# embedded-software-laboratory/p-dmpc

Measured on AMD Instinct MI355X. Metric: MPC steps/sec (whole node) + p50 per-step plan latency, N vehicles H=8, higher is better.
Workload: dtype f64

## Files before the change

p-dmpc_amd/csrc/api.cpp:

```cpp
#include <hip/hip_runtime.h>

#include <algorithm>
#include <cmath>
#include <cstdio>
#include <cstdlib>
#include <chrono>
#include <cstring>
#include <limits>
#include <mutex>
#include <string>
#include <type_traits>
#include <vector>

#include "choice_host.hpp"
#include "handle.hpp"
#include "mpa_reach.hpp"
#include "reference_tree.hpp"
#include "sampled_launch.hpp"

namespace {

thread_local std::string g_err;

std::mutex g_lds_mutex;
uint32_t g_lds_high_water[64][4][2];

void set_launch_args(pdmpc_handle* h, const PackedStep& B, const LaunchPlan& plan, int first, int count, KernelArgs& a) {
    set_batch_args(h, B, plan.areas_in_lds, a);
    set_plan_args(h->tune, plan, a);
    a.dt = h->cfg.dt_seconds;
    a.max_nodes = h->arena.max_nodes;
    a.checker = h->cfg.checker;
    a.pred = B.dev.pred;
    a.done_flag = h->d_flag.p;
    a.epoch = h->epoch;
    a.first = first;
    a.arena = h->arena.view();
    a.soup_cap = B.soup_cap;
    a.cand_cap = B.cand_cap;
    a.tie_count = h->d_tie_count.p;
    if (h->tune.debug_progress && !h->progress) {
        if (hipHostMalloc((void**)&h->progress, (size_t)h->max_vehicles * 64 * 4, hipHostMallocMapped) != hipSuccess) h->progress = nullptr;
        if (h->progress) std::memset(h->progress, 0, (size_t)h->max_vehicles * 64 * 4);
    }
    a.progress = h->progress;
    a.bk_post = h->d_bk_post.p;
    a.help_board = h->d_help_board.p;
    a.help_verdict = h->d_help_verdict.p;
    a.help_finished = h->d_help_finished.p;
    h->launch_serial += 1;
    if (h->launch_serial == 0) h->launch_serial = 1;
    a.launch_id = h->launch_serial;
    a.n_searches = count;
}

int prepare_boards(pdmpc_handle* h, int count, uint32_t& fin_base) {
    fin_base = 0;
    if (!h->boards_dirty) {
        fin_base = h->help_fin_total;
        h->help_fin_total += (uint32_t)count;
    } else {
        HIPCHK(hipMemsetAsync(h->d_help_board.p, 0, (size_t)h->max_vehicles * PDMPC_HB_WORDS * sizeof(unsigned long long), h->stream));
        HIPCHK(hipMemsetAsync(h->d_help_finished.p, 0, 16 * sizeof(uint32_t), h->stream));
        h->help_fin_total = (uint32_t)count;
        h->boards_dirty = false;
    }
    return PDMPC_OK;
}

struct SearchLaunch {
    KernelArgs a{};

    int prepare(pdmpc_handle* h, const PackedStep& B, int first, int count, bool safe, LaunchPlan& plan) {
        const LaunchDims dims = launch_dims(h, B);
        int n_chained = 0;
        if (!safe && policy_reads_chained(h->tune, count, dims.n_cu, dims.device_share))
            for (int i = 0; i < count; ++i) n_chained += B.host.veh[first + i].n_pred > 0 ? 1 : 0;
        std::string err;
        int rc = plan_launch(h->tune, dims, kPlanSearch, count, n_chained, safe, plan, err);
        if (rc) return fail(rc, err);
        set_launch_args(h, B, plan, first, count, a);
        if (plan.n_helpers > 0 && (rc = prepare_boards(h, count, a.help_fin_base))) return rc;
        if (h->tune.debug_lds) fputs(format_bulk_layout(plan, count).c_str(), stderr);
        return PDMPC_OK;
    }

    int go(const pdmpc_handle* h, const LaunchPlan& plan) const {
        typedef int (*launcher_t)(const KernelArgs*, int, void*, uint32_t*);
        static const launcher_t launchers[4][2] = {{pdmpc_launch_bulk, pdmpc_launch_bulk_any},
                                                   {pdmpc_launch_bulk_wide, pdmpc_launch_bulk_wide_any},
                                                   {pdmpc_launch_bulk_sat, pdmpc_launch_bulk_sat_any},
                                                   {pdmpc_launch_bulk_compact, pdmpc_launch_bulk_compact_any}};
        const int variant = plan.variant, generic = plan.generic ? 1 : 0;
        int lrc = 0;
        for (int done = 0; done < a.n_searches && lrc == 0; done += plan.slice) {
            KernelArgs part = a;
            part.first = a.first + done;
            part.n_searches = std::min(plan.slice, a.n_searches - done);
            std::lock_guard<std::mutex> lock(g_lds_mutex);
            lrc = launchers[variant][generic](&part, part.n_searches, (void*)h->stream, &g_lds_high_water[h->cfg.device & 63][variant][generic]);
        }
        return lrc;
    }
};

template <class Launch>
int timed_launch(pdmpc_handle* h, const PackedStep& B, int first, int count, bool safe, LaunchKind kind) {
    LaunchPlan plan;
    Launch launch;
    int rc = launch.prepare(h, B, first, count, safe, plan);
    if (rc) return rc;
    if ((rc = h->timer.begin(h->stream, kind))) return rc;
    const int lrc = launch.go(h, plan);
    if (lrc != 0) {
        h->boards_dirty = true;
        char buf[256];
        snprintf(buf, sizeof buf, "kernel launch failed: %s (LDS %u B)", hipGetErrorString((hipError_t)lrc), plan.lds.total);
        return fail(PDMPC_ERR_HIP, buf);
    }
    if ((rc = h->timer.end(h->stream))) return rc;
    h->stats.lds_bytes = plan.lds.total;
    h->stats.lds_nodes = plan.NL;
    return PDMPC_OK;
}

int launch_range(pdmpc_handle* h, int first, int count, bool safe) {
    if (!h) return fail(PDMPC_ERR_INVALID, "null handle");
    PackedStep& B = h->banks[h->bank];
// ... 1133 lines not shown
```

p-dmpc_amd/csrc/bulk_search.hpp:

```cpp
#include <hip/hip_runtime.h>

#include "search_common.hpp"

#include "frontier_common.hpp"

#include "bk_shared.hpp"
#include "bk_helper.hpp"

#define BK_P2 3
#define BK_PER PDMPC_BK_PER
#define BK_FAST_PER 4

namespace {

__device__ __forceinline__ unsigned long long wg_scan_excl(unsigned long long v, lds_vu64* wsum, int lane, int wave, int n_waves, unsigned long long& total) {
    unsigned long long inc = v;
#pragma unroll
    for (int o = 1; o < PDMPC_WAVE; o <<= 1) {
        const unsigned long long t = __shfl_up(inc, o);
        inc += lane >= o ? t : 0ull;
    }
    if (lane == PDMPC_WAVE - 1) wsum[wave] = inc;
    __syncthreads();
    unsigned long long off = 0, tot = 0;
// ... 1492 lines not shown
                    if (bsel != 0u || scale == 0.0 || (to_mid ? cum <= 4u * fill : nn_near + cum <= OC - 64u)) break;
                    hi = lo + (hi - lo) / (double)FR_NBINS;
                }
                const bool all = bsel >= FR_NBINS - 1 || scale == 0.0;
                const double l_new = all ? inf : lo + (double)(bsel + 1u) / scale;
                if (tid == 0) {
                    if (from_mid) {
                        sh_st_d(sh, BK_MID_MIN, inf);
                    } else {
                        sh_st_d(sh, FR_FAR_MIN, inf);
                        sh_st_d(sh, FR_FAR_MAX, 0.0);
                    }
                    if (to_mid) {
                        sh_st_d(sh, BK_L_MID, all ? hi_src : l_new);
                    } else {
                        if (!from_mid) sh_st_d(sh, BK_L_MID, -1.0);
                        if (nn_near == 0u) {
                            sh_st_d(sh, FR_NEAR_MIN, inf);
                            sh_st_d(sh, FR_NEAR_MAX, 0.0);
                        }
                        const double l_far_new = (all && far_left != 0u) ? l_mid_old : l_new;
                        const double l_old = sh_ld_d(sh, FR_L_FAR);
                        sh_st_d(sh, FR_L_FAR, (nn_near != 0u && l_old > l_far_new && l_old < inf) ? l_old : l_far_new);
                    }
                }
                __syncthreads();
                load_l_mid();
                const double lo_c = lo, scale_c = scale;
                const uint32_t kept = fr_partition(
                    src_key, src_id, fn, wsum, n_waves, [&](double k, uint32_t i) -> int { return i == 0u ? -1 : (fr_bin(k, lo_c, scale_c) <= bsel ? 1 : 0); },
                    [&](int c, double k, uint32_t i) {
                        const unsigned long long b = __ballot(c == 1);
                        bool back = false;
                        if (b && to_mid) {
                            const uint32_t base = sh_add_uniform(sh, BK_MID_N, (uint32_t)__builtin_popcountll(b), lane);
                            if (c == 1) {
                                const uint32_t pos = base + lane_rank(b, lane);
                                mid_key[pos] = k;
                                mid_id[pos] = i;
                                mid_mn = k < mid_mn ? k : mid_mn;
                            }
                        } else if (b) {
                            const uint32_t base = sh_add_uniform(sh, FR_NEAR_N, (uint32_t)__builtin_popcountll(b), lane);
                            const uint32_t pos = base + lane_rank(b, lane);
                            const bool fits = c == 1 && pos < OC;
                            if (fits) {
                                near_key[pos] = k;
                                near_id[pos] = i;
                                near_mn = k < near_mn ? k : near_mn;
                                near_mx = k > near_mx ? k : near_mx;
                            }
                            back = c == 1 && !fits;
                        }
                        if (!to_mid) to_far(back, k, i);
                        if (c < 0 && i != 0u) {
                            if (from_mid) {
                                mid_mn = k < mid_mn ? k : mid_mn;
                            } else {
                                far_mn = k < far_mn ? k : far_mn;
                                far_mx = k > far_mx ? k : far_mx;
                            }
                        }
                    });
                flush_far();
                flush_near();
                const uint32_t extra = sh[SRC_N] - fn;
                for (uint32_t e = (uint32_t)tid; e < extra; e += (uint32_t)bd) {
                    src_key[kept + e] = src_key[fn + e];
                    src_id[kept + e] = src_id[fn + e];
                }
                asm volatile("s_waitcnt vmcnt(0)" ::: "memory");
                __syncthreads();
                if (tid == 0) {
                    sh[SRC_N] = kept + extra;
                    if (sh[FR_NEAR_N] > OC) sh[FR_NEAR_N] = OC;
                }
                __syncthreads();
            }
            nn_near = sh[FR_NEAR_N];
            BK_TICK(tk_refill)
        }

        BK_OPAQUE_TID
        if (nn_near <= (uint32_t)(BK_FAST_PER * PDMPC_WAVE)) {
            BK_TICK3(4)
            __syncthreads();
            if (wave == 0) {
                const double lo = sh_ld_d(sh, FR_NEAR_MIN), hi = sh_ld_d(sh, FR_NEAR_MAX);
                double kk[BK_FAST_PER];
                uint32_t ii[BK_FAST_PER];
#pragma unroll
                for (int j = 0; j < BK_FAST_PER; ++j) {
                    const uint32_t e = (uint32_t)j * PDMPC_WAVE + (uint32_t)lane;
                    kk[j] = e < nn_near ? near_key[e] : 0.0;
                    ii[j] = e < nn_near ? near_id[e] : 0u;
                }
                double thr = hi;
                if (nn_near > round_target) {
                    double a = lo, b = hi;
                    for (int it = 0; it < 48; ++it) {
                        const double mid = a + (b - a) * 0.5;
                        if (!(mid > a) || !(mid < b)) break;
                        uint32_t c = 0;
#pragma unroll
                        for (int j = 0; j < BK_FAST_PER; ++j) c += (uint32_t)__builtin_popcountll(__ballot(ii[j] != 0u && kk[j] <= mid));
                        if (c >= round_target) {
                            thr = mid;
                            b = mid;
                            if (c <= 2u * round_target + 16u) break;
                        } else {
                            a = mid;
                        }
                    }
                }
                const bool have_goal = best != 0u;
                const bool check_alive = sh[FR_EVER_INVAL] != 0u;
                const uint32_t epoch_now = sh[BK_ARRIVALS] & 0xffffu;
                ulonglong2* const wcache = (ulonglong2*)A.arena.walk + voff;
                uint32_t pk = 0, pr = 0, n_dead = 0, n_drop = 0;
#pragma unroll
                for (int j = 0; j < BK_FAST_PER; ++j) {
                    const double k = kk[j];
                    const uint32_t i = ii[j];
                    const bool sel = i != 0u && k <= thr;
                    const bool above = have_goal && k > bb;
                    const bool walk = sel && !above && (have_goal || check_alive);
                    if (sel && have_goal && k == bb) atomicOr((uint32_t*)&sh[FR_FLAGS], FRF_TIE);
                    int r = 1;
                    if (have_goal || check_alive) r = bk_classify_wave(F.glink, wcache, VS, F.gkey, gp_path, gp_mp, have_goal, check_alive, best, epoch_now, walk ? i : 0u, k, sh);
                    const int c = i == 0u ? -1 : (sel ? (above ? 3 : r) : 0);
                    const unsigned long long bk = __ballot(c == 0), br = __ballot(c == 1);
                    n_dead += (uint32_t)__builtin_popcountll(__ballot(c == 4));
                    n_drop += (uint32_t)__builtin_popcountll(__ballot(c == 3));
                    if (c == 0) {
                        const uint32_t pos = pk + lane_rank(bk, lane);
                        near_key[pos] = k;
                        near_id[pos] = i;
                        near_mn = k < near_mn ? k : near_mn;
                        near_mx = k > near_mx ? k : near_mx;
                    } else if (c == 1) {
                        const uint32_t pos = pr + lane_rank(br, lane);
                        ready[pos] = i;
                        r_flag[pos] = 0u;
                    }
                    pk += (uint32_t)__builtin_popcountll(bk);
                    pr += (uint32_t)__builtin_popcountll(br);
                }
                if (lane == 0) {
                    sh[FR_NEAR_N] = pk;
                    sh_st_d(sh, FR_NEAR_MIN, inf);
                    sh_st_d(sh, FR_NEAR_MAX, 0.0);
                    sh[FR_SEL_BIN] = pr;
                    if (n_dead) sh[FR_DEAD] = sh[FR_DEAD] + n_dead;
                    if (n_drop) sh[FR_DROPPED] = sh[FR_DROPPED] + n_drop;
                }
            }
            __syncthreads();
            Rn = sh[FR_SEL_BIN];
            BK_TICK3(5)
            BK_TICK(tk_select)
            continue;
        }
        {
            BK_TICK3(4)
            if (!(nn_near > round_target)) __syncthreads();
            const double lo = sh_ld_d(sh, FR_NEAR_MIN);
            double hi = sh_ld_d(sh, FR_NEAR_MAX);
            double kk[BK_PER];
            uint32_t ii[BK_PER];
#pragma unroll
            for (int j = 0; j < BK_PER; ++j) {
                const uint32_t e = (uint32_t)j * (uint32_t)bd + (uint32_t)tid;
                kk[j] = e < nn_near ? near_key[e] : 0.0;
                ii[j] = e < nn_near ? near_id[e] : 0u;
            }
            uint32_t bsel = BK_NB - 1;
            double scale = 0.0;
            const bool use_hist = nn_near > round_target;
            if (use_hist) {
                for (int zoom = 0; zoom < 8; ++zoom) {
                    scale = hi > lo ? (double)BK_NB / (hi - lo) : 0.0;
#pragma unroll
                    for (int j = 0; j < BK_PER; ++j)
                        if (ii[j]) __hip_atomic_fetch_add(&bins[bk_bin(kk[j], lo, scale)], 1u, __ATOMIC_RELAXED, __HIP_MEMORY_SCOPE_WORKGROUP);
                    __syncthreads();
                    uint32_t cum;
                    bk_select(bins, round_target, lane, bsel, cum);
                    if (cum <= 2u * round_target + 16u || scale == 0.0) break;
                    hi = lo + (hi - lo) / (double)BK_NB;
                    __syncthreads();
                    if (tid < BK_NB) bins[tid] = 0u;
                    __syncthreads();
                }
            }
            const bool have_goal = best != 0u;
            const bool check_alive = sh[FR_EVER_INVAL] != 0u;
            const uint32_t epoch_now = sh[BK_ARRIVALS] & 0xffffu;
            ulonglong2* const wcache = (ulonglong2*)A.arena.walk + voff;
            int cls[BK_PER];
            unsigned long long mine = 0;
            uint32_t n_dead = 0, n_drop = 0;
#pragma unroll
            for (int j = 0; j < BK_PER; ++j) {
                const double k = kk[j];
                const uint32_t i = ii[j];
                const uint32_t b = bk_bin(k, lo, scale);
                const bool sel = i != 0u && b <= bsel;
                const bool above = have_goal && k > bb;
                const bool walk = sel && !above && (have_goal || check_alive);
                if (sel && have_goal && k == bb) atomicOr((uint32_t*)&sh[FR_FLAGS], FRF_TIE);
                int r = 1;
                if (have_goal || check_alive) r = bk_classify_wave(F.glink, wcache, VS, F.gkey, gp_path, gp_mp, have_goal, check_alive, best, epoch_now, walk ? i : 0u, k, sh);
                cls[j] = i == 0u ? -1 : (sel ? (above ? 3 : r) : 0);
                mine += (cls[j] == 0 ? 1ull : 0ull) | (cls[j] == 1 ? (1ull << 32) : 0ull);
                n_dead += cls[j] == 4 ? 1u : 0u;
                n_drop += cls[j] == 3 ? 1u : 0u;
            }
            unsigned long long tot = 0;
            const unsigned long long base = wg_scan_excl(mine, wsum64 + 16, lane, wave, n_waves, tot);
            if (use_hist && tid < BK_NB) bins[tid] = 0u;
            const uint32_t n_keep = (uint32_t)(tot & 0xffffffffull), n_rdy = (uint32_t)(tot >> 32);
            if (tid == 0) {
                sh[FR_NEAR_N] = n_keep;
                sh_st_d(sh, FR_NEAR_MIN, inf);
                sh_st_d(sh, FR_NEAR_MAX, 0.0);
            }
            {
                uint32_t pk = (uint32_t)(base & 0xffffffffull), pr = (uint32_t)(base >> 32);
                bool over[BK_PER];
#pragma unroll
                for (int j = 0; j < BK_PER; ++j) {
                    over[j] = false;
                    if (cls[j] == 0) {
                        near_key[pk] = kk[j];
                        near_id[pk] = ii[j];
                        near_mn = kk[j] < near_mn ? kk[j] : near_mn;
                        near_mx = kk[j] > near_mx ? kk[j] : near_mx;
                        pk += 1u;
                    } else if (cls[j] == 1) {
                        if (pr < RC) {
                            ready[pr] = ii[j];
                            r_flag[pr] = 0u;
                        } else {
                            over[j] = true;
                        }
                        pr += 1u;
                    }
                }
                if (n_rdy > RC) {
#pragma unroll
                    for (int j = 0; j < BK_PER; ++j) to_far(over[j], kk[j], ii[j]);
                }
            }
            if (n_dead) sh_add(sh, FR_DEAD, n_dead);
            if (n_drop) sh_add(sh, FR_DROPPED, n_drop);
            Rn = n_rdy < RC ? n_rdy : RC;
            __syncthreads();
            BK_TICK3(5)
            BK_TICK(tk_select)
        }
    }

    int tid_r = tid_k, lane_r = lane_k;
    asm volatile("" : "+v"(tid_r), "+v"(lane_r));
    uint32_t nnodes_raw = sh[FR_NNODES];
    nnodes_raw = nnodes_raw < S.max_nodes ? nnodes_raw : S.max_nodes;
    __syncthreads();
    const bool pb_ran = pb_valid;
    if (!pb_valid) {
        R.n_popped = 0;
        R.n_expanded = nnodes_raw;
    }
    {
        const uint32_t nv = vs_copied ? 0u : (VS.NV < nnodes_raw ? VS.NV : nnodes_raw);
        for (uint32_t i = (uint32_t)tid_r; i < nv; i += (uint32_t)bd) VS.g[i] = VS.l[i];
    }
    {
        unsigned long long a = t_checks, b = t_pairs;
#pragma unroll
        for (int o = PDMPC_WAVE / 2; o > 0; o >>= 1) {
            a += __shfl_xor(a, o);
            b += __shfl_xor(b, o);
        }
        if (lane_r == 0) {
            atomicAdd(A.work_count + 0, a);
            atomicAdd(A.work_count + 1, b);
        }
    }
    if (tid_r == 0) {
        atomicAdd(P.counters + 2, (int)sh[BK_ARRIVALS]);
        atomicAdd(A.work_count + 2, (unsigned long long)sh[FR_PROCESSED]);
        atomicAdd(A.work_count + 3, (unsigned long long)sh[FR_ROUNDS]);
        A.tree_size[slot] = (int32_t)(nnodes_raw | PDMPC_TREE_FRONTIER | (tie_replayed ? PDMPC_TREE_REPLAYED : 0u));
    }
    if (tid_r == 0 && SW::debug_tail(A)) {
        double* dbg = X.O->path_nodes[PDMPC_HP_MAX];
        dbg[0] = (double)sh[FR_ROUNDS];
        dbg[1] = (double)sh[FR_PROCESSED];
        dbg[2] = (double)nnodes_raw;
        dbg[3] = (double)sh[FR_NEAR_N];
        dbg[4] = (double)(sh[FR_FAR_N] + sh[BK_MID_N]);
        dbg[5] = (double)sh[FR_FLAGS];
        dbg[6] = (double)sh[BK_ARRIVALS];
        dbg[7] = (double)(__builtin_amdgcn_s_memrealtime() - tk[TK_START]);
        for (int i = 0; i < 6; ++i) X.O->path_nodes[PDMPC_HP_MAX - 3][i] = (double)tk2[i];
        if (A.n_helpers > 0) {
            const unsigned long long sw = __hip_atomic_load(board + PDMPC_HB_SEATS, __ATOMIC_RELAXED, __HIP_MEMORY_SCOPE_AGENT);
            X.O->path_nodes[PDMPC_HP_MAX - 3][7] = (double)pdmpc_hb_seats_count(sw);
        }
        X.O->path_nodes[PDMPC_HP_MAX - 2][0] = (double)(tk[TK_START] - X.rt_kernel_start);
        X.O->path_nodes[PDMPC_HP_MAX - 2][1] = (double)tk[tk_p1];
        X.O->path_nodes[PDMPC_HP_MAX - 2][2] = (double)tk[tk_p2];
        X.O->path_nodes[PDMPC_HP_MAX - 2][3] = (double)tk[tk_p3];
        X.O->path_nodes[PDMPC_HP_MAX - 2][4] = (double)tk[tk_pb];
        X.O->path_nodes[PDMPC_HP_MAX - 2][5] = (double)tk[tk_refill];
        X.O->path_nodes[PDMPC_HP_MAX - 1][0] = (double)(tk[tk_work] + tk[tk_p1] + tk[tk_p2] + tk[tk_p3]);
        X.O->path_nodes[PDMPC_HP_MAX - 1][1] = (double)tk[tk_arrival];
        X.O->path_nodes[PDMPC_HP_MAX - 1][2] = (double)tk[tk_select];
        X.O->path_nodes[PDMPC_HP_MAX - 1][3] = (double)tk[tk_wait];
        X.O->path_nodes[PDMPC_HP_MAX - 1][4] = (double)(tk[TK_MARK] - tk[TK_START]);
        X.O->path_nodes[PDMPC_HP_MAX - 1][5] = (double)tk[tk_pub];
        X.O->path_nodes[PDMPC_HP_MAX - 1][6] = (double)__builtin_amdgcn_s_memrealtime();
        X.O->path_nodes[PDMPC_HP_MAX - 1][7] = (double)X.rt_kernel_start;
    }
    X.status = status;
    X.n_popped = (int)R.n_popped;
    X.path_ready = pb_ran && goal != 0u;
    X.goal = goal;
    X.nnodes = R.n_expanded;
    X.dep_timeout = dep_timeout;
    X.rec_valid = rec_valid && !dep_timeout;
    X.rec_written = rec_written;
    X.published = sh[BK_PUBLISHED] != 0u;
}

template <int NW, int CHECKER, class SW>
__device__ __forceinline__ void bulk_body(const KernelArgs& A) {
    if ((int)blockIdx.x < A.bk_helpers_first || (int)blockIdx.x >= A.bk_helpers_first + A.n_searches) {
        bulk_helper_body<CHECKER, SW>(A);
        return;
    }
    extern __shared__ __attribute__((aligned(16))) unsigned char smem[];
    Ctx X;
    const unsigned long long rt0 = __builtin_amdgcn_s_memrealtime();
    search_prologue<SW>(A, X, (LDS_AS unsigned char*)smem);
    X.rt_kernel_start = rt0;
    const int wave = X.wave;
    lds_u32* ref_ids = bk_misc(X.lsm)->ref_ids;
    bulk_search<NW, CHECKER, SW>(A, X, ref_ids);
    __syncthreads();
    if (wave != 0) return;
    {
        int l__ = X.lane;
        asm volatile("" : "+v"(l__));
        X.lane = l__;
    }
    if (!X.rec_valid) bk_write_record(A, X, X.goal, X.status, X.dep_timeout, (uint32_t)X.n_popped, X.nnodes, X.path_ready, ref_ids, X.rec_written, X.published, X.lane);
    bk_publish(A, X, X.status, X.dep_timeout);
    if (X.lane == 0 && A.n_helpers > 0) {
        __hip_atomic_store(A.help_board + (size_t)X.slot * PDMPC_HB_WORDS + PDMPC_HB_WANT, 0ull, __ATOMIC_RELAXED, __HIP_MEMORY_SCOPE_AGENT);
        atomicAdd(A.help_finished, 1u);
    }
}

}

#ifndef PDMPC_BULK_KERNEL_ATTR
#define PDMPC_BULK_KERNEL_ATTR
#endif
#define PDMPC_BULK_INSTANCE(NAME, LAUNCHER, NW, CHECKER, MAXWAVES, SW)                                                                   \
    extern "C" __global__ __launch_bounds__(PDMPC_WAVE * (MAXWAVES)) PDMPC_BULK_KERNEL_ATTR void NAME(const KernelArgs A) { bulk_body<NW, CHECKER, SW>(A); } \
    extern "C" int LAUNCHER(const KernelArgs* args, int count, void* stream, uint32_t* lds_high_water) {                                \
        if (count <= 0) return 0;                                                                                                        \
        typedef void (*kernel_t)(const KernelArgs);                                                                                      \
        kernel_t fn = NAME;                                                                                                              \
         \
        uint32_t& have = lds_high_water[0];                                                                                              \
        if (args->lds.total > have) {                                                                                                    \
            hipError_t e = hipFuncSetAttribute((const void*)fn, hipFuncAttributeMaxDynamicSharedMemorySize, (int)args->lds.total);       \
            if (e != hipSuccess) return (int)e;                                                                                          \
            have = args->lds.total;                                                                                                      \
        }                                                                                                                                \
        hipLaunchKernelGGL(fn, dim3(count + (args->n_helpers > 0 ? args->n_helpers : 0)), dim3(PDMPC_WAVE * args->n_waves), args->lds.total, (hipStream_t)stream, *args); \
        return (int)hipGetLastError();                                                                                                   \
    }
#define PDMPC_BULK_KERNEL(NAME, LAUNCHER, NW, CHECKER, MAXWAVES, KERNEL)                    \
    PDMPC_BULK_INSTANCE(NAME, LAUNCHER, NW, CHECKER, MAXWAVES, SwitchesProduct<KERNEL>)  \
    PDMPC_BULK_INSTANCE(NAME##_any, LAUNCHER##_any, NW, CHECKER, MAXWAVES, SwitchesFromArgs)
```

p-dmpc_amd/csrc/handle.hpp:

```cpp
#pragma once
#include <vector>

#include "hdv_host.hpp"
#include "hip_host.hpp"
#include "launch_plan.hpp"
#include "pdmpc_device.h"


struct Arenas {
    uint32_t max_nodes = 0;
    DevBuf<NodeRec> nodes;
    DevBuf<double> key, far_key, mid_key, pb_key, walk;
    DevBuf<unsigned long long> link;
    DevBuf<uint32_t> far_id, mid_id, pb_d, child0, vlist;
    DevBuf<uint8_t> vstate;
    template <class Self, class F>
    static void each(Self& a, int Hp, F&& f) {
        f(a.nodes, 1);
        f(a.key, 1);
        f(a.link, 1);
        f(a.vstate, 1);
        f(a.far_key, 1);
        f(a.far_id, 1);
        f(a.mid_key, 1);
        f(a.mid_id, 1);
        f(a.pb_key, 1);
        f(a.pb_d, 1);
        f(a.walk, 2);
        f(a.child0, 1);
        f(a.vlist, Hp + 1);
    }
    size_t bytes_per_node(int Hp) const {
        size_t sum = 0;
        each(*this, Hp, [&](const auto& b, int per) { sum += (size_t)per * sizeof *b.p; });
        return sum;
    }
    int alloc(int max_vehicles, uint32_t n, int Hp) {
        n = (n + 1u) & ~1u;
        const size_t tot = (size_t)max_vehicles * n;
        each(*this, Hp, [](auto& b, int) { b.release(); });
        max_nodes = 0;
        int bad = 0;
        each(*this, Hp, [&](auto& b, int per) { bad |= b.ensure_exact(tot * (size_t)per); });
        if (bad) return bad;
        max_nodes = n;
        return 0;
    }
    NodeArena view() const {
        return {nodes.p, key.p, link.p, vstate.p, far_key.p, far_id.p, mid_key.p, mid_id.p, pb_key.p, pb_d.p, walk.p, child0.p, vlist.p};
    }
};

enum LaunchKind : int32_t { kLaunchSearch = 2, kLaunchSampled = 3, kLaunchJoint = 4 };

struct BlobRegions {
    DevVehicle* veh = nullptr;
    int32_t* pred = nullptr;
    double* pts = nullptr;
};

struct PackedStep {
    PinnedBuf<unsigned char> h_blob;
    DevBuf<unsigned char> d_blob;
    BlobRegions host, dev;
    uint64_t staged_serial = ~0ull;
    int n_packed = 0;
    bool pack_failed = false;
    SampledBank sampled;
    int soup_cap = 0;
    int ll_cap = 0;
    int cand_cap = 0;
    std::vector<int64_t> lit_cols;
    std::vector<int32_t> perm;
    std::vector<int32_t> inv;
};

struct SoupKey {
    const void* p[13];
    int32_t c[6];
};

struct SoupTable {
    std::vector<SoupKey> keys;
    std::vector<int32_t> slot;
    std::vector<int32_t> table;
    static uint64_t hash(const SoupKey& k) {
        static_assert(sizeof(SoupKey) % 8 == 0, "SoupKey is hashed by 64-bit words");
        uint64_t hsh = 1469598103934665603ull;
        const uint64_t* w = (const uint64_t*)&k;
        for (size_t q = 0; q < sizeof(SoupKey) / 8; ++q) hsh = (hsh ^ w[q]) * 1099511628211ull;
        return hsh ^ (hsh >> 29);
    }
    void reset(int n) {
        size_t size = 64;
        while (size < (size_t)n * 2) size *= 2;
        keys.clear();
        slot.clear();
        table.assign(size, 0);
    }
    int find(const SoupKey& k, size_t& at) const {
        for (at = (size_t)hash(k) & (table.size() - 1); table[at] != 0; at = (at + 1) & (table.size() - 1)) {
            const int q = table[at] - 1;
            if (std::memcmp(&keys[(size_t)q], &k, sizeof k) == 0) return slot[(size_t)q];
        }
        return -1;
    }
    void insert(const SoupKey& k, int packed_in, size_t at) {
        keys.push_back(k);
        slot.push_back(packed_in);
        table[at] = (int32_t)keys.size();
    }
};

struct LaunchTimer {
    static constexpr size_t kMaxPairs = 4096;
    std::vector<std::pair<hipEvent_t, hipEvent_t>> events;
    size_t used = 0;
    double folded_ms = 0.0;
    int64_t folded_launches = 0;
    LaunchKind kind = kLaunchSampled;
    LaunchTimer() = default;
    LaunchTimer(const LaunchTimer&) = delete;
    LaunchTimer& operator=(const LaunchTimer&) = delete;
    ~LaunchTimer() { release(); }
    void release() {
        for (auto& ev : events) {
            (void)hipEventDestroy(ev.first);
            (void)hipEventDestroy(ev.second);
        }
        events.clear();
        used = 0;
    }
// ... 244 lines not shown
```

p-dmpc_amd/csrc/pdmpc_device.h:

```cpp
#ifndef PDMPC_DEVICE_H
#define PDMPC_DEVICE_H

#include <stdint.h>

#include "../../include/pdmpc.h"
#include "../../include/pdmpc_hdv.h"

#define PDMPC_WAVE 64
#define PDMPC_MAX_WAVES 16
#define PDMPC_MAX_WAVES_SAT 12
#define PDMPC_SH_WORDS 128

struct DevManPose {
    double dx, dy, dyaw;
    int32_t n_cols;
    int32_t pad;
};

struct DevVehicle {
    double x0, y0, yaw0;
    double ref_x[PDMPC_HP_MAX];
    double ref_y[PDMPC_HP_MAX];
    double v_ref[PDMPC_HP_MAX];
    int32_t trim0;
    int32_t n_pred;
    int32_t pred_off;
    int32_t ll_off, ll_len;
    int32_t lit_off[PDMPC_HP_MAX + 1];
    int32_t hdv_off[PDMPC_HP_MAX + 1];
    int32_t fb_off[PDMPC_HP_MAX + 1];
    uint32_t seed;
};

struct NodeRec {
    double x, y, yaw, g;
    double cs, sn;
    double h;
    uint32_t parent;
    uint32_t packed;
};
#define NODE_TRIM(p) ((int)((p) & 1023u))
#define NODE_K(p) ((int)(((p) >> 10) & 31u))
#define NODE_MAN(p) ((int)(((p) >> 15) & 4095u))
#define NODE_COLS(p) ((int)(((p) >> 27) & 15u))

struct LdsLayout {
    uint32_t mask, man_index, pose, area;
    uint32_t ref;
    uint32_t shape;
    uint32_t path;
    uint32_t soup;
    uint32_t cand;
    uint32_t vstate;
    uint32_t expand;
    uint32_t tree16;
    uint32_t rand;
    uint32_t nodes;
    uint32_t total;
    uint32_t bk_near_key, bk_near_id;
    uint32_t bk_ready;
    uint32_t bk_hist;
    uint32_t bk_misc;
    uint32_t bk_pshape;
    uint32_t reach_shared;
    uint32_t bk_reach;
    uint32_t reach;
};

struct LdsPathRegion {
    uint32_t path[PDMPC_HP_MAX + 2];
    int32_t soff[PDMPC_HP_MAX + 1];
    int32_t hoff[PDMPC_HP_MAX + 1];
    uint32_t shared[PDMPC_SH_WORDS];
    int32_t lit[PDMPC_HP_MAX];
};
#define PDMPC_LK_PATH_BYTES PDMPC_LK_ALIGN16((uint32_t)sizeof(LdsPathRegion))

#define PDMPC_LK_ALIGN16(x) (((x) + 15u) & ~15u)
#ifndef PDMPC_LK_WAVES
#define PDMPC_LK_WAVES PDMPC_MAX_WAVES
#endif
#ifndef PDMPC_LK_READY_CAP
#define PDMPC_LK_READY_CAP 2048u
#endif
#define PDMPC_LK_COMPACT_WAVES 8
#define PDMPC_LK_COMPACT_READY_CAP 512u
#define PDMPC_LK_COMPACT_BK_PER 2
#define PDMPC_LKX_THREADS(W) ((uint32_t)(W) * PDMPC_WAVE)
#define PDMPC_LKX_REF 0u
#define PDMPC_LKX_SHAPE (PDMPC_LKX_REF + 3u * PDMPC_HP_MAX * 8u)
#define PDMPC_LKX_PATH(W) (PDMPC_LKX_SHAPE + (uint32_t)(W) * (2u * PDMPC_VMAX + 1u) * 16u)
#define PDMPC_LKX_CAND(W) (PDMPC_LKX_PATH(W) + PDMPC_LK_PATH_BYTES)
#define PDMPC_LKX_EXPAND(W) (PDMPC_LKX_CAND(W) + PDMPC_LK_ALIGN16(12u * PDMPC_LKX_THREADS(W)))
#define PDMPC_LKX_NEAR_KEY(W) (PDMPC_LKX_EXPAND(W) + (2u * PDMPC_HP_MAX * PDMPC_HP_MAX) * 8u + 16u * 16u)
#define PDMPC_LKX_NEAR_ID(W, P) (PDMPC_LKX_NEAR_KEY(W) + PDMPC_LK_ALIGN16((uint32_t)(P) * PDMPC_LKX_THREADS(W) * 8u))
#define PDMPC_LKX_READY(W, P) (PDMPC_LKX_NEAR_ID(W, P) + PDMPC_LK_ALIGN16((uint32_t)(P) * PDMPC_LKX_THREADS(W) * 4u))
#define PDMPC_LKX_HIST(W, RC, P) (PDMPC_LKX_READY(W, P) + (uint32_t)(RC) * 8u)
#define PDMPC_LKX_MISC(W, RC, P) (PDMPC_LKX_HIST(W, RC, P) + 3072u * 4u)
#define PDMPC_LKX_PSHAPE(W, RC, P) (PDMPC_LKX_MISC(W, RC, P) + 2048u)
#define PDMPC_LKX_REACH(W, RC, P) (PDMPC_LKX_PSHAPE(W, RC, P) + PDMPC_LK_ALIGN16(PDMPC_HP_MAX * PDMPC_VMAX * 16u + PDMPC_HP_MAX * 4u + PDMPC_HP_MAX * 8u + PDMPC_HP_MAX * 4u))
#define PDMPC_LK_REACH_CNT (PDMPC_HP_MAX * 4u * 8u)
#define PDMPC_LK_REACH_STALE (PDMPC_LK_REACH_CNT + 3u * PDMPC_HP_MAX * 4u)
#define PDMPC_LK_REACH_SC (PDMPC_LK_REACH_STALE + 16u)
#define PDMPC_LK_REACH_ROOT (PDMPC_LK_REACH_SC + 32u)
#define PDMPC_LKX_FIXED_END(W, RC, P) (PDMPC_LKX_REACH(W, RC, P) + PDMPC_LK_REACH_ROOT + 64u)
#ifndef PDMPC_BK_PER
#define PDMPC_BK_PER 4
#endif
#define PDMPC_LK_REF PDMPC_LKX_REF
#define PDMPC_LK_SHAPE PDMPC_LKX_SHAPE
#define PDMPC_LK_PATH PDMPC_LKX_PATH(PDMPC_LK_WAVES)
#define PDMPC_LK_CAND PDMPC_LKX_CAND(PDMPC_LK_WAVES)
#define PDMPC_LK_EXPAND PDMPC_LKX_EXPAND(PDMPC_LK_WAVES)
#define PDMPC_LK_NEAR_KEY PDMPC_LKX_NEAR_KEY(PDMPC_LK_WAVES)
#define PDMPC_LK_NEAR_ID PDMPC_LKX_NEAR_ID(PDMPC_LK_WAVES, PDMPC_BK_PER)
#define PDMPC_LK_READY PDMPC_LKX_READY(PDMPC_LK_WAVES, PDMPC_BK_PER)
#define PDMPC_LK_HIST PDMPC_LKX_HIST(PDMPC_LK_WAVES, PDMPC_LK_READY_CAP, PDMPC_BK_PER)
#define PDMPC_LK_MISC PDMPC_LKX_MISC(PDMPC_LK_WAVES, PDMPC_LK_READY_CAP, PDMPC_BK_PER)
#define PDMPC_LK_PSHAPE PDMPC_LKX_PSHAPE(PDMPC_LK_WAVES, PDMPC_LK_READY_CAP, PDMPC_BK_PER)
#define PDMPC_LK_REACH PDMPC_LKX_REACH(PDMPC_LK_WAVES, PDMPC_LK_READY_CAP, PDMPC_BK_PER)
#define PDMPC_LK_FIXED_END PDMPC_LKX_FIXED_END(PDMPC_LK_WAVES, PDMPC_LK_READY_CAP, PDMPC_BK_PER)

struct NodeArena {
    NodeRec* nodes;
    double* key;
    unsigned long long* link;
    uint8_t* vstate;
    double* far_key;
    uint32_t* far_id;
    double* mid_key;
    uint32_t* mid_id;
    double* pb_key;
    uint32_t* pb_d;
    double* walk;
    uint32_t* child0;
    uint32_t* vlist;
};

static inline uint32_t pdmpc_lk_fixed(uint32_t W, uint32_t RC, uint32_t P, LdsLayout* L) {
    L->ref = PDMPC_LKX_REF;
    L->shape = PDMPC_LKX_SHAPE;
    L->path = PDMPC_LKX_PATH(W);
    L->cand = PDMPC_LKX_CAND(W);
    L->expand = PDMPC_LKX_EXPAND(W);
    L->bk_near_key = PDMPC_LKX_NEAR_KEY(W);
    L->bk_near_id = PDMPC_LKX_NEAR_ID(W, P);
    L->bk_ready = PDMPC_LKX_READY(W, P);
    L->bk_hist = PDMPC_LKX_HIST(W, RC, P);
    L->bk_misc = PDMPC_LKX_MISC(W, RC, P);
    L->bk_pshape = PDMPC_LKX_PSHAPE(W, RC, P);
    L->bk_reach = PDMPC_LKX_REACH(W, RC, P);
    return PDMPC_LKX_FIXED_END(W, RC, P);
}

#define PDMPC_HELP_CAP 2048
#define PDMPC_HB_SEATS_MAX 64
#define PDMPC_HB_N 1
#define PDMPC_HB_MASK 2
#define PDMPC_HB_SEATS 3
#define PDMPC_HB_WANT 4
#define PDMPC_HB_WEIGHT 5
#define PDMPC_HB_ASSIGN 8
#define PDMPC_HB_DONE 72
#define PDMPC_HB_WORDS 136
#define PDMPC_VALUE_FN constexpr __attribute__((always_inline)) inline
#define PDMPC_HB_ASSIGN_WORD(round, first, count) (((unsigned long long)(round) << 40) | ((unsigned long long)(first) << 20) | (unsigned long long)(count))
PDMPC_VALUE_FN unsigned long long pdmpc_hb_assign(uint32_t round, uint32_t first, uint32_t count) { return PDMPC_HB_ASSIGN_WORD(round, first, count); }
PDMPC_VALUE_FN uint32_t pdmpc_hb_assign_round(unsigned long long w) { return (uint32_t)(w >> 40); }
PDMPC_VALUE_FN uint32_t pdmpc_hb_assign_first(unsigned long long w) { return (uint32_t)((w >> 20) & 0xfffffull); }
PDMPC_VALUE_FN uint32_t pdmpc_hb_assign_count(unsigned long long w) { return (uint32_t)(w & 0xfffffull); }
PDMPC_VALUE_FN unsigned long long pdmpc_hb_seats(uint32_t launch_id, uint32_t taken) { return ((unsigned long long)launch_id << 32) | (unsigned long long)taken; }
PDMPC_VALUE_FN uint32_t pdmpc_hb_seats_launch(unsigned long long w) { return (uint32_t)(w >> 32); }
PDMPC_VALUE_FN unsigned long long pdmpc_hb_seats_count(unsigned long long w) { return w & 0xffffffffull; }
#define PDMPC_HB_SEATS_TAKEN(w, launch_id) ((uint32_t)((w) >> 32) == (launch_id) ? (uint32_t)((w) & 0xffffffffull) : 0u)
PDMPC_VALUE_FN uint32_t pdmpc_hb_seats_taken(unsigned long long w, uint32_t launch_id) { return PDMPC_HB_SEATS_TAKEN(w, launch_id); }
PDMPC_VALUE_FN uint32_t pdmpc_hb_verdict(uint32_t flags) { return (flags & 1u) ? 2u : ((flags & 2u) ? 3u : 1u); }
PDMPC_VALUE_FN bool pdmpc_hb_verdict_missing(uint32_t v) { return v < 1u || v > 3u; }
PDMPC_VALUE_FN uint32_t pdmpc_hb_verdict_flags(uint32_t v) { return v == 2u ? 1u : (v == 3u ? 2u : 0u); }
#define PDMPC_ALL_PREDECESSORS(n_pred) ((n_pred) >= 64 ? ~0ull : ((1ull << (n_pred)) - 1ull))
PDMPC_VALUE_FN unsigned long long pdmpc_all_predecessors(int n_pred) { return PDMPC_ALL_PREDECESSORS(n_pred); }
PDMPC_VALUE_FN bool pdmpc_hb_assign_round_trips(uint32_t round, uint32_t first, uint32_t count) {
    return pdmpc_hb_assign_round(pdmpc_hb_assign(round, first, count)) == round && pdmpc_hb_assign_first(pdmpc_hb_assign(round, first, count)) == first &&
           pdmpc_hb_assign_count(pdmpc_hb_assign(round, first, count)) == count;
}
static_assert(PDMPC_HELP_CAP < (1 << 20), "a first entry and an entry count each fit their 20 bits of the assignment word");
static_assert(pdmpc_hb_assign_round_trips(0u, 0u, 0u) && pdmpc_hb_assign_round_trips(1u, 1u, 1u) && pdmpc_hb_assign_round_trips(1u, PDMPC_HELP_CAP, PDMPC_HELP_CAP) &&
                  pdmpc_hb_assign_round_trips((1u << 24) - 1u, (1u << 20) - 1u, (1u << 20) - 1u) && pdmpc_hb_assign_round_trips((1u << 24) - 1u, 0u, 0u) &&
                  pdmpc_hb_assign_round_trips(0u, (1u << 20) - 1u, 0u) && pdmpc_hb_assign_round_trips(0u, 0u, (1u << 20) - 1u),
              "the fields of the assignment word do not overlap");
static_assert(pdmpc_hb_assign_round(pdmpc_hb_assign(1u << 24, 0u, 0u)) == 0u, "the round is cut to 24 bits");
static_assert(pdmpc_hb_seats_taken(pdmpc_hb_seats(7u, 0u), 7u) == 0u && pdmpc_hb_seats_taken(pdmpc_hb_seats(7u, 0u) + 3ull, 7u) == 3u && pdmpc_hb_seats_taken(pdmpc_hb_seats(7u, 5u), 8u) == 0u &&
                  pdmpc_hb_seats_taken(pdmpc_hb_seats(0xffffffffu, PDMPC_HB_SEATS_MAX), 0xffffffffu) == PDMPC_HB_SEATS_MAX,
              "a seat is counted for its own launch only");
static_assert(pdmpc_hb_verdict(0u) == 1u && pdmpc_hb_verdict(1u) == 2u && pdmpc_hb_verdict(2u) == 3u && pdmpc_hb_verdict(3u) == 2u, "a crossing of a real area decides");
static_assert(pdmpc_hb_verdict_flags(1u) == 0u && pdmpc_hb_verdict_flags(2u) == 1u && pdmpc_hb_verdict_flags(3u) == 2u && pdmpc_hb_verdict_missing(0u) && pdmpc_hb_verdict_missing(4u) &&
                  !pdmpc_hb_verdict_missing(1u) && !pdmpc_hb_verdict_missing(3u),
              "the owner reads a verdict back as the flag bits P2 expects");
static_assert(pdmpc_all_predecessors(0) == 0ull && pdmpc_all_predecessors(1) == 1ull && pdmpc_all_predecessors(63) == 0x7fffffffffffffffull && pdmpc_all_predecessors(64) == ~0ull &&
                  pdmpc_all_predecessors(65) == ~0ull,
              "one bit per predecessor, all 64 from 64 on");

struct KernelArgs {
    const uint64_t* succ_mask;
    const int16_t* man_index;
    const DevManPose* man_pose;
    const double* man_area;
    int32_t n_trims, n_words, n_man, Hp;
    int32_t checker;
    int32_t areas_in_lds;
    double dt;
    const DevVehicle* veh;
    const double* points;
    const int32_t* pred;
    pdmpc_vehicle_out* out;
    uint32_t* done_flag;
    uint32_t epoch;
    int32_t first;
    NodeArena arena;
    uint32_t max_nodes;
    int32_t* tree_size;
#define PDMPC_TREE_FRONTIER 0x40000000
#define PDMPC_TREE_REPLAYED 0x20000000
#define PDMPC_TREE_SIZE(sz) ((sz) & ~(PDMPC_TREE_FRONTIER | PDMPC_TREE_REPLAYED))
    LdsLayout lds;
    int32_t NL, NV, soup_cap, cand_cap;
    int32_t n_waves;
    unsigned long long* work_count;
    int32_t* tie_count;
    uint32_t* progress;
    int32_t debug_tail;
    int32_t n_searches;
    int32_t n_helpers;
    unsigned long long* help_board;
    uint32_t* help_verdict;
    uint32_t* help_finished;
    uint32_t help_fin_base;
    uint32_t launch_id;
    int32_t bk_ready_cap;
    int32_t bk_round0;
    int32_t bk_round;
    int32_t bk_ramp;
    int32_t bk_helpers_first;
    int32_t bk_seat_nodes;
    int32_t bk_tentative;
    int32_t bk_tile;
    int32_t bk_mid_min;
    int32_t bk_mid_fill;
    int32_t bk_share_min;
    int32_t bk_force_tie;
    int32_t bk_fast_arrival;
    double* bk_post;
    int32_t speculate;
    uint32_t spin_limit;
    int32_t reverse_dispatch;
};

enum { PDMPC_BULK = 0, PDMPC_BULK_WIDE = 1, PDMPC_BULK_SAT = 2, PDMPC_BULK_COMPACT = 3 };
struct ProductSwitches {
    static constexpr int32_t debug_tail = 0, bk_force_tie = 0, reverse_dispatch = 0, bk_tentative = 1, bk_fast_arrival = 1, speculate = 1;
    static constexpr int32_t areas_in_lds(int kernel) { return kernel == PDMPC_BULK || kernel == PDMPC_BULK_SAT ? 1 : 0; }
    static bool matches(const KernelArgs& a, int kernel) {
        return a.debug_tail == debug_tail && a.bk_force_tie == bk_force_tie && a.reverse_dispatch == reverse_dispatch && a.bk_tentative == bk_tentative &&
               a.bk_fast_arrival == bk_fast_arrival && a.speculate == speculate && a.areas_in_lds == areas_in_lds(kernel);
    }
};

struct JointLds {
    uint32_t mask, man_index, pose, area;
    uint32_t ref;
    uint32_t shape;
    uint32_t ints;
    uint32_t succ;
    uint32_t soup;
    uint32_t heap_key, heap_id;
    uint32_t total;
};
#define PDMPC_JOINT_INTS (PDMPC_JOINT_MAX * (PDMPC_HP_MAX + 1) + 3 * PDMPC_JOINT_MAX + PDMPC_HP_MAX + 1)

#ifdef __HIP__
#define PDMPC_HOST_DEVICE __attribute__((host)) __attribute__((device))
#else
#define PDMPC_HOST_DEVICE
#endif
PDMPC_HOST_DEVICE static inline int pdmpc_joint_soup_owner(const DevVehicle* veh, int v, int Hp) {
    for (int u = 0; u < v; ++u) {
        bool same = true;
        for (int k = 0; k <= Hp && same; ++k) same = veh[u].lit_off[k] == veh[v].lit_off[k];
        if (same) return u;
    }
    return -1;
}
PDMPC_HOST_DEVICE static inline int pdmpc_joint_boundary_owner(const DevVehicle* veh, int v) {
    for (int u = 0; u < v; ++u)
        if (veh[u].ll_off == veh[v].ll_off && veh[u].ll_len == veh[v].ll_len) return u;
    return -1;
}
PDMPC_HOST_DEVICE static inline int pdmpc_joint_soup_columns(const DevVehicle* veh, int N, int Hp) {
    int need = 0;
    for (int v = 0; v < N; ++v) {
        if (pdmpc_joint_soup_owner(veh, v, Hp) < 0) need += veh[v].lit_off[Hp] - veh[v].lit_off[0];
        if (pdmpc_joint_boundary_owner(veh, v) < 0) need += veh[v].ll_len;
    }
    return need;
}

struct JointArgs {
    const uint64_t* succ_mask;
    const int16_t* man_index;
    const DevManPose* man_pose;
    const double* man_area;
    int32_t n_trims, n_words, n_man, Hp;
    int32_t areas_in_lds;
    double dt;
    const DevVehicle* veh;
    const double* points;
    const int32_t* problem_off;
    pdmpc_vehicle_out* out;
    NodeRec* nodes;
    double* far_key;
    uint32_t* far_id;
    uint32_t max_nodes;
    uint32_t heap_lds;
    int32_t* tree_size;
    unsigned long long* work_count;
    JointLds lds;
};

#define PDMPC_PRIO_MAX_N 64
#define PDMPC_PRIO_MAX_E 32
#define PDMPC_PRIO_THREADS 256
#define PDMPC_PRIO_ROUNDS 16
#define PDMPC_PRIO_TILE (PDMPC_PRIO_THREADS * PDMPC_PRIO_ROUNDS)
struct PriorityArgs {
    uint32_t in_base[PDMPC_PRIO_MAX_N];
    uint32_t out_base[PDMPC_PRIO_MAX_N];
    int32_t active[PDMPC_PRIO_MAX_N];
    int32_t n, E, n_active;
    uint32_t all_edges;
// ... 246 lines not shown
```

Baseline: 1618.

## Group hot kernel arguments into cache blocks and pin them in scalar registers

Reorders KernelArgs, NodeArena and LdsLayout so the fields read in the search's round loop sit in contiguous 32-byte blocks at the front of the kernel-argument segment, with static_asserts fixing the layout. In bulk_body the hot fields are copied from the kernarg pointer into scalar registers through inline asm, so they are not reloaded from memory inside the loop. The goal flag is rebuilt per iteration from an opaque register copy of best. The progress debug pointer is removed from the arguments; this saves space but drops debug progress output, and the inline asm may raise scalar register pressure.

```diff
diff --git a/p-dmpc_amd/csrc/api.cpp b/p-dmpc_amd/csrc/api.cpp
--- a/p-dmpc_amd/csrc/api.cpp
+++ b/p-dmpc_amd/csrc/api.cpp
@@ -43,7 +43,6 @@
         if (hipHostMalloc((void**)&h->progress, (size_t)h->max_vehicles * 64 * 4, hipHostMallocMapped) != hipSuccess) h->progress = nullptr;
         if (h->progress) std::memset(h->progress, 0, (size_t)h->max_vehicles * 64 * 4);
     }
-    a.progress = h->progress;
     a.bk_post = h->d_bk_post.p;
     a.help_board = h->d_help_board.p;
     a.help_verdict = h->d_help_verdict.p;
diff --git a/p-dmpc_amd/csrc/bulk_search.hpp b/p-dmpc_amd/csrc/bulk_search.hpp
--- a/p-dmpc_amd/csrc/bulk_search.hpp
+++ b/p-dmpc_amd/csrc/bulk_search.hpp
@@ -1598,6 +1598,10 @@
         }
 
         BK_OPAQUE_TID
+#define BK_HAVE_GOAL                          \
+    uint32_t best_own = best;                 \
+    asm volatile("" : "+v"(best_own));        \
+    const bool have_goal = best_own != 0u;
         if (nn_near <= (uint32_t)(BK_FAST_PER * PDMPC_WAVE)) {
             BK_TICK3(4)
             __syncthreads();
@@ -1629,13 +1633,13 @@
                         }
                     }
                 }
-                const bool have_goal = best != 0u;
                 const bool check_alive = sh[FR_EVER_INVAL] != 0u;
                 const uint32_t epoch_now = sh[BK_ARRIVALS] & 0xffffu;
                 ulonglong2* const wcache = (ulonglong2*)A.arena.walk + voff;
                 uint32_t pk = 0, pr = 0, n_dead = 0, n_drop = 0;
 #pragma unroll
                 for (int j = 0; j < BK_FAST_PER; ++j) {
+                    BK_HAVE_GOAL
                     const double k = kk[j];
                     const uint32_t i = ii[j];
                     const bool sel = i != 0u && k <= thr;
@@ -1643,7 +1647,7 @@
                     const bool walk = sel && !above && (have_goal || check_alive);
                     if (sel && have_goal && k == bb) atomicOr((uint32_t*)&sh[FR_FLAGS], FRF_TIE);
                     int r = 1;
-                    if (have_goal || check_alive) r = bk_classify_wave(F.glink, wcache, VS, F.gkey, gp_path, gp_mp, have_goal, check_alive, best, epoch_now, walk ? i : 0u, k, sh);
+                    if (have_goal || check_alive) r = bk_classify_wave(F.glink, wcache, VS, F.gkey, gp_path, gp_mp, have_goal, check_alive, best_own, epoch_now, walk ? i : 0u, k, sh);
                     const int c = i == 0u ? -1 : (sel ? (above ? 3 : r) : 0);
                     const unsigned long long bk = __ballot(c == 0), br = __ballot(c == 1);
                     n_dead += (uint32_t)__builtin_popcountll(__ballot(c == 4));
@@ -1709,7 +1713,6 @@
                     __syncthreads();
                 }
             }
-            const bool have_goal = best != 0u;
             const bool check_alive = sh[FR_EVER_INVAL] != 0u;
             const uint32_t epoch_now = sh[BK_ARRIVALS] & 0xffffu;
             ulonglong2* const wcache = (ulonglong2*)A.arena.walk + voff;
@@ -1718,6 +1721,7 @@
             uint32_t n_dead = 0, n_drop = 0;
 #pragma unroll
             for (int j = 0; j < BK_PER; ++j) {
+                BK_HAVE_GOAL
                 const double k = kk[j];
                 const uint32_t i = ii[j];
                 const uint32_t b = bk_bin(k, lo, scale);
@@ -1726,7 +1730,7 @@
                 const bool walk = sel && !above && (have_goal || check_alive);
                 if (sel && have_goal && k == bb) atomicOr((uint32_t*)&sh[FR_FLAGS], FRF_TIE);
                 int r = 1;
-                if (have_goal || check_alive) r = bk_classify_wave(F.glink, wcache, VS, F.gkey, gp_path, gp_mp, have_goal, check_alive, best, epoch_now, walk ? i : 0u, k, sh);
+                if (have_goal || check_alive) r = bk_classify_wave(F.glink, wcache, VS, F.gkey, gp_path, gp_mp, have_goal, check_alive, best_own, epoch_now, walk ? i : 0u, k, sh);
                 cls[j] = i == 0u ? -1 : (sel ? (above ? 3 : r) : 0);
                 mine += (cls[j] == 0 ? 1ull : 0ull) | (cls[j] == 1 ? (1ull << 32) : 0ull);
                 n_dead += cls[j] == 4 ? 1u : 0u;
@@ -1851,16 +1855,39 @@
 }
 
 template <int NW, int CHECKER, class SW>
-__device__ __forceinline__ void bulk_body(const KernelArgs& A) {
-    if ((int)blockIdx.x < A.bk_helpers_first || (int)blockIdx.x >= A.bk_helpers_first + A.n_searches) {
-        bulk_helper_body<CHECKER, SW>(A);
+__device__ __forceinline__ void bulk_body(const KernelArgs& A_kernel) {
+    if ((int)blockIdx.x < A_kernel.bk_helpers_first || (int)blockIdx.x >= A_kernel.bk_helpers_first + A_kernel.n_searches) {
+        bulk_helper_body<CHECKER, SW>(A_kernel);
         return;
     }
     extern __shared__ __attribute__((aligned(16))) unsigned char smem[];
     Ctx X;
     const unsigned long long rt0 = __builtin_amdgcn_s_memrealtime();
-    search_prologue<SW>(A, X, (LDS_AS unsigned char*)smem);
+    search_prologue<SW>(A_kernel, X, (LDS_AS unsigned char*)smem);
     X.rt_kernel_start = rt0;
+    KernelArgs A = A_kernel;
+    typedef const __attribute__((address_space(4))) KernelArgs* bk_kargs_ptr;
+    bk_kargs_ptr kp = (bk_kargs_ptr)__builtin_amdgcn_kernarg_segment_ptr();
+    asm volatile("" : "+s"(kp));
+#define BK_OWN(field)                                                                              \
+    {                                                                                              \
+        decltype(A.field) own__;                                                                   \
+        if constexpr (sizeof(own__) == 4) {                                                        \
+            asm volatile("s_mov_b32 %0, %1" : "=s"(own__) : "s"(kp->field));                       \
+        } else {                                                                                   \
+            static_assert(sizeof(own__) == 8, "a kernel argument is one or two scalar registers"); \
+            asm volatile("s_mov_b64 %0, %1" : "=s"(own__) : "s"(kp->field));                       \
+        }                                                                                          \
+        A.field = own__;                                                                           \
+    }
+    BK_OWN(out) BK_OWN(done_flag) BK_OWN(pred) BK_OWN(epoch) BK_OWN(first)
+    BK_OWN(points) BK_OWN(veh) BK_OWN(man_area) BK_OWN(work_count)
+    BK_OWN(bk_ready_cap)
+    BK_OWN(spin_limit) BK_OWN(n_helpers) BK_OWN(launch_id) BK_OWN(help_board) BK_OWN(help_verdict)
+    BK_OWN(bk_post) BK_OWN(tie_count) BK_OWN(max_nodes) BK_OWN(arena.walk) BK_OWN(arena.child0) BK_OWN(arena.vlist)
+    BK_OWN(arena.link) BK_OWN(arena.far_key) BK_OWN(arena.far_id) BK_OWN(arena.mid_key) BK_OWN(arena.mid_id) BK_OWN(arena.pb_key) BK_OWN(arena.pb_d)
+    BK_OWN(tree_size) BK_OWN(help_finished)
+#undef BK_OWN
     const int wave = X.wave;
     lds_u32* ref_ids = bk_misc(X.lsm)->ref_ids;
     bulk_search<NW, CHECKER, SW>(A, X, ref_ids);
diff --git a/p-dmpc_amd/csrc/handle.hpp b/p-dmpc_amd/csrc/handle.hpp
--- a/p-dmpc_amd/csrc/handle.hpp
+++ b/p-dmpc_amd/csrc/handle.hpp
@@ -47,7 +47,7 @@
         return 0;
     }
     NodeArena view() const {
-        return {nodes.p, key.p, link.p, vstate.p, far_key.p, far_id.p, mid_key.p, mid_id.p, pb_key.p, pb_d.p, walk.p, child0.p, vlist.p};
+        return {walk.p, child0.p, vlist.p, nodes.p, key.p, link.p, vstate.p, far_key.p, far_id.p, mid_key.p, mid_id.p, pb_key.p, pb_d.p};
     }
 };
 
diff --git a/p-dmpc_amd/csrc/pdmpc_device.h b/p-dmpc_amd/csrc/pdmpc_device.h
--- a/p-dmpc_amd/csrc/pdmpc_device.h
+++ b/p-dmpc_amd/csrc/pdmpc_device.h
@@ -1,6 +1,7 @@
 #ifndef PDMPC_DEVICE_H
 #define PDMPC_DEVICE_H
 
+#include <stddef.h>
 #include <stdint.h>
 
 #include "../../include/pdmpc.h"
@@ -46,23 +47,23 @@
 
 struct LdsLayout {
     uint32_t mask, man_index, pose, area;
+    uint32_t soup;
+    uint32_t vstate;
+    uint32_t nodes;
+    uint32_t reach_shared;
     uint32_t ref;
     uint32_t shape;
     uint32_t path;
-    uint32_t soup;
     uint32_t cand;
-    uint32_t vstate;
     uint32_t expand;
     uint32_t tree16;
     uint32_t rand;
-    uint32_t nodes;
     uint32_t total;
     uint32_t bk_near_key, bk_near_id;
     uint32_t bk_ready;
     uint32_t bk_hist;
     uint32_t bk_misc;
     uint32_t bk_pshape;
-    uint32_t reach_shared;
     uint32_t bk_reach;
     uint32_t reach;
 };
@@ -122,6 +123,9 @@
 #define PDMPC_LK_FIXED_END PDMPC_LKX_FIXED_END(PDMPC_LK_WAVES, PDMPC_LK_READY_CAP, PDMPC_BK_PER)
 
 struct NodeArena {
+    double* walk;
+    uint32_t* child0;
+    uint32_t* vlist;
     NodeRec* nodes;
     double* key;
     unsigned long long* link;
@@ -132,9 +136,6 @@
     uint32_t* mid_id;
     double* pb_key;
     uint32_t* pb_d;
-    double* walk;
-    uint32_t* child0;
-    uint32_t* vlist;
 };
 
 static inline uint32_t pdmpc_lk_fixed(uint32_t W, uint32_t RC, uint32_t P, LdsLayout* L) {
@@ -201,59 +202,72 @@
               "one bit per predecessor, all 64 from 64 on");
 
 struct KernelArgs {
+    pdmpc_vehicle_out* out;
+    uint32_t* done_flag;
+    const int32_t* pred;
+    uint32_t epoch;
+    int32_t first;
+    const double* points;
+    const DevVehicle* veh;
+    const double* man_area;
+    unsigned long long* work_count;
+    int32_t bk_round0;
+    int32_t bk_round;
+    int32_t bk_ramp;
+    int32_t bk_ready_cap;
+    int32_t bk_mid_min;
+    int32_t bk_mid_fill;
+    int32_t bk_share_min;
+    int32_t bk_tile;
+    uint32_t spin_limit;
+    int32_t n_helpers;
+    uint32_t launch_id;
+    int32_t areas_in_lds;
+    unsigned long long* help_board;
+    uint32_t* help_verdict;
+    double* bk_post;
+    int32_t* tie_count;
+    uint32_t max_nodes;
+    int32_t bk_fast_arrival;
+    NodeArena arena;
     const uint64_t* succ_mask;
     const int16_t* man_index;
     const DevManPose* man_pose;
-    const double* man_area;
+    double dt;
     int32_t n_trims, n_words, n_man, Hp;
     int32_t checker;
-    int32_t areas_in_lds;
-    double dt;
-    const DevVehicle* veh;
-    const double* points;
-    const int32_t* pred;
-    pdmpc_vehicle_out* out;
-    uint32_t* done_flag;
-    uint32_t epoch;
-    int32_t first;
-    NodeArena arena;
-    uint32_t max_nodes;
+    int32_t NL, NV, soup_cap;
+    int32_t cand_cap;
+    int32_t n_waves;
+    int32_t n_searches;
+    int32_t bk_helpers_first;
+    int32_t bk_tentative;
+    int32_t speculate;
+    int32_t reverse_dispatch;
+    int32_t bk_force_tie;
+    LdsLayout lds;
     int32_t* tree_size;
 #define PDMPC_TREE_FRONTIER 0x40000000
 #define PDMPC_TREE_REPLAYED 0x20000000
 #define PDMPC_TREE_SIZE(sz) ((sz) & ~(PDMPC_TREE_FRONTIER | PDMPC_TREE_REPLAYED))
-    LdsLayout lds;
-    int32_t NL, NV, soup_cap, cand_cap;
-    int32_t n_waves;
-    unsigned long long* work_count;
-    int32_t* tie_count;
-    uint32_t* progress;
-    int32_t debug_tail;
-    int32_t n_searches;
-    int32_t n_helpers;
-    unsigned long long* help_board;
-    uint32_t* help_verdict;
     uint32_t* help_finished;
     uint32_t help_fin_base;
-    uint32_t launch_id;
-    int32_t bk_ready_cap;
-    int32_t bk_round0;
-    int32_t bk_round;
-    int32_t bk_ramp;
-    int32_t bk_helpers_first;
     int32_t bk_seat_nodes;
-    int32_t bk_tentative;
-    int32_t bk_tile;
-    int32_t bk_mid_min;
-    int32_t bk_mid_fill;
-    int32_t bk_share_min;
-    int32_t bk_force_tie;
-    int32_t bk_fast_arrival;
-    double* bk_post;
-    int32_t speculate;
-    uint32_t spin_limit;
-    int32_t reverse_dispatch;
-};
+    int32_t debug_tail;
+};
+#define PDMPC_ARGS_BLOCK 32
+#define PDMPC_ARGS_HOT_END offsetof(KernelArgs, succ_mask)
+#define PDMPC_ARGS_COLD_BEGIN offsetof(KernelArgs, tree_size)
+static_assert(offsetof(KernelArgs, out) == 0 && offsetof(KernelArgs, points) == 1 * PDMPC_ARGS_BLOCK && offsetof(KernelArgs, bk_round0) == 2 * PDMPC_ARGS_BLOCK &&
+                  offsetof(KernelArgs, spin_limit) == 3 * PDMPC_ARGS_BLOCK && offsetof(KernelArgs, bk_post) == 4 * PDMPC_ARGS_BLOCK,
+              "every group of round-loop fields -- arrivals, record and lists, selection, sharing, arenas -- begins a 32-byte block");
+static_assert(offsetof(KernelArgs, arena) + sizeof(NodeArena) == PDMPC_ARGS_HOT_END && PDMPC_ARGS_HOT_END == 8 * PDMPC_ARGS_BLOCK, "the round loop's fields end with a block");
+static_assert(offsetof(KernelArgs, arena.walk) / PDMPC_ARGS_BLOCK == offsetof(KernelArgs, bk_post) / PDMPC_ARGS_BLOCK, "the walk cache's pointer shares the block of the posted entries'");
+static_assert(offsetof(KernelArgs, lds) % PDMPC_ARGS_BLOCK == 0 && sizeof(LdsLayout) % PDMPC_ARGS_BLOCK == 0 && offsetof(LdsLayout, ref) == PDMPC_ARGS_BLOCK,
+              "the layout begins a block, ends with one, and the offsets a search's prologue reads are its first block");
+static_assert(PDMPC_ARGS_COLD_BEGIN == offsetof(KernelArgs, lds) + sizeof(LdsLayout) && PDMPC_ARGS_COLD_BEGIN % PDMPC_ARGS_BLOCK == 0 && PDMPC_ARGS_COLD_BEGIN == 14 * PDMPC_ARGS_BLOCK,
+              "the prologue's fields end with a block");
+static_assert(sizeof(KernelArgs) == 15 * PDMPC_ARGS_BLOCK, "KernelArgs is fifteen 32-byte blocks: eight of the round loop, six of the prologue, one of the rest");
 
 enum { PDMPC_BULK = 0, PDMPC_BULK_WIDE = 1, PDMPC_BULK_SAT = 2, PDMPC_BULK_COMPACT = 3 };
 struct ProductSwitches {
```

New measurement: 1611. No clear change (-0.4%).
